# Jonetz/TreeDetection

Measured on AMD Instinct MI355X. Metric: tiles/sec (1000x1000 RGB+nDSM) predict_tiles model stage, higher is better.
Workload: dtype f32

## Files before the change

treedetection_amd/csrc/api.cpp:

```cpp
#include "common.h"
#include "detect.h"
#include <cstdarg>
#include <cstdio>
#include <cmath>
#include <cstdlib>
#include <vector>


namespace {
td_status scratch(void** p, size_t bytes) {
    TD_HIP_CHECK(hipMalloc(p, bytes ? bytes : 16));
    return TD_OK;
}
}

extern "C" {

void td_model_desc_default(td_model_desc* d) {
    d->num_classes = 1;
    d->precision = TD_PRECISION_FP32;
    d->pre_nms_topk = 1000;
    d->post_nms_topk = 1000;
    d->detections_per_image = 100;
    d->rpn_nms_thresh = 0.7f;
// ... 36 lines not shown
    a.stride = 1; a.pad = pad;
    a.Ho = H + 2 * pad - KH + 1;
    a.Wo = W + 2 * pad - KW + 1;
    a.relu = 1; a.M = B * a.Ho * a.Wo; a.m_mul = 1;
    a.tile_cfg = ((precision >> 8) & 0xff) - 1;
    TD_REQUIRE(conv_head_capable(a.tile_cfg, TD_PRECISION_FP16), "td_conv2d_head_nhwc: tile id %d does not own 256 output channels per block", a.tile_cfg);
    a.head_w = head_w; a.head_b = head_b; a.head_y = head_y; a.head_n = head_n;
    a.y = head_y;
    return conv2d_api(a, precision, stream);
}

static td_status conv2d_api(ConvArgs& a, int precision, void* stream) {
    hipStream_t s = static_cast<hipStream_t>(stream);
    ConvArgs with_frag = a;
    with_frag.w_frag = a.w;
    if (!conv_tile(a.tile_cfg) || !conv_tile(a.tile_cfg)->frag || conv_tile_refusal(a.tile_cfg, with_frag, precision & 0xff))
        return conv2d_launch(a, precision & 0xff, s);
    const int es = (precision & 0xff) == TD_PRECISION_FP16 ? 2 : 4;
    const size_t n = (size_t)a.Cout * a.KH * a.KW * a.Cin;
    std::vector<unsigned char> bits(n * es), packed;
    TD_HIP_CHECK(hipStreamSynchronize(s));
    TD_HIP_CHECK(hipMemcpy(bits.data(), a.w, n * es, hipMemcpyDeviceToHost));
    conv_bd_pack(bits.data(), es, a.Cout, a.KH, a.KW, a.Cin, packed);
    void* wf = nullptr;
    td_status st = scratch(&wf, packed.size());
    if (st < 0) return st;
    hipError_t herr = hipMemcpy(wf, packed.data(), packed.size(), hipMemcpyHostToDevice);
    a.w_frag = wf;
    if (herr == hipSuccess) st = conv2d_launch(a, precision & 0xff, s);
    hipError_t herr2 = hipStreamSynchronize(s);
// ... 212 lines not shown
```

treedetection_amd/csrc/common.h:

```cpp
#pragma once
#include <hip/hip_runtime.h>
#include <hip/hip_fp16.h>
#include <cstdint>
#include <cstddef>
#include "../../include/treedet.h"
#include <string>
#include <vector>

void td_set_error(const char* fmt, ...);

int td_polygons_json_text(const int32_t* mask_region, const int64_t* mask_offset, const uint32_t* mask_bits, int64_t mask_words,
                          const float* scores, const int32_t* classes, int n, const double* transform, const char* image_id,
                          std::string& out, const char* who);

#define TD_HIP_CHECK(expr)                                                                         \
    do {                                                                                           \
        hipError_t _e = (expr);                                                                    \
        if (_e != hipSuccess) {                                                                    \
            td_set_error("%s failed: %s (%s:%d)", #expr, hipGetErrorString(_e), __FILE__, __LINE__); \
            return TD_ERR_HIP;                                                                     \
        }                                                                                          \
    } while (0)

#define TD_REQUIRE(cond, ...)            \
// ... 17 lines not shown
    const float* bias;
    const void* res;
    void* y;
    int B, H, W, Cin, Cout, KH, KW, stride, pad, Ho, Wo;
    int res_shift;
    int relu;
    int out_mode;
    int M;
    const int* m_dyn;
    int m_mul;
    int m_off;
    int out_f32;
    int batch_count;
    long long x_bs, w_bs, y_bs;
    const void* w_frag;
    int tile_cfg;
    int tile_strict;
    const void* head_w;
    const float* head_b;
    float* head_y;
    int head_n;
    int nlev;
    struct Level {
        const void* x;
        const void* w;
        const float* bias;
        void* y;
        float* head_y;
        int H, W, M, tile0;
    } lev[5];
    int ntiles;
};
enum ConvFamily : unsigned char { TILE_IGEMM, TILE_PP8, TILE_PLANE, TILE_BD, TILE_BS, TILE_RETIRED };
enum : unsigned char { TILE_F32 = 1 << TD_PRECISION_FP32, TILE_F16 = 1 << TD_PRECISION_FP16, TILE_ANY = TILE_F32 | TILE_F16 };
struct ConvTile {
    ConvFamily family;
    unsigned char variant;
    unsigned char prec;
    bool head;
    bool frag;
    signed char tune_rank;
    unsigned char max_ksteps;
    short min_cout, max_cout;
};
inline constexpr ConvTile TD_CONV_TILES[] = {
    {TILE_IGEMM,   0, TILE_ANY, false, false,  5, 0,   0,  0},
    {TILE_IGEMM,   0, TILE_ANY, false, false, 10, 0,   0,  0},
    {TILE_IGEMM,   0, TILE_ANY, false, false, 11, 0,   0,  0},
// ... 16 lines not shown
    {TILE_PLANE,   0, TILE_F32, false, false, 19, 0,   0,  0},
    {TILE_PLANE,   0, TILE_F32, false, false, 20, 0,   0,  0},
    {TILE_RETIRED, 0, 0,        false, false, -1, 0,   0,  0},
    {TILE_RETIRED, 0, 0,        false, false, -1, 0,   0,  0},
    {TILE_BD,      0, TILE_ANY, true,  true,   8, 0,   0,  0},
    {TILE_BD,      1, TILE_ANY, false, true,  12, 0,   0,  0},
    {TILE_BD,      2, TILE_ANY, false, true,  13, 0,   0,  0},
    {TILE_BD,      3, TILE_ANY, false, true,  14, 0,   0,  0},
    {TILE_BD,      4, TILE_ANY, true,  true,   9, 0,   0,  0},
    {TILE_RETIRED, 0, 0,        false, false, -1, 0,   0,  0},
    {TILE_BD,      5, TILE_ANY, true,  true,   3, 0,   0,  0},
    {TILE_BD,      6, TILE_ANY, false, true,   7, 0,   0,  0},
    {TILE_IGEMM,   0, TILE_ANY, false, false, 15, 0,   0, 32},
    {TILE_IGEMM,   0, TILE_ANY, false, false, 17, 0,   0, 32},
    {TILE_BS,      0, TILE_ANY, false, true,   0, 4, 128,  0},
};
static inline const ConvTile* conv_tile(int id) { return id >= 0 && id < (int)(sizeof TD_CONV_TILES / sizeof *TD_CONV_TILES) ? &TD_CONV_TILES[id] : nullptr; }
static inline bool conv_head_capable(int id, int precision) { return precision == TD_PRECISION_FP16 && conv_tile(id) && conv_tile(id)->head; }
const char* conv_tile_refusal(int id, const ConvArgs& a, int precision);
td_status conv2d_launch(const ConvArgs& a, int precision, hipStream_t stream);
td_status conv_pp8_grouped_launch(ConvArgs a, hipStream_t stream);
void conv_bd_pack(const void* w_ohwi, int elem_bytes, int cout, int kh, int kw, int cin, std::vector<unsigned char>& out);
bool conv_bd_ok(const ConvArgs& a, int precision);
td_status conv_bd_launch(const ConvArgs& a, int precision, int variant, hipStream_t stream);
bool conv_bs_ok(const ConvArgs& a, int precision);
td_status conv_bs_launch(const ConvArgs& a, int precision, hipStream_t stream);
td_status wino_gemm_launch(const ConvArgs& a, hipStream_t stream);

struct TailArgs {
    const void* x;
    const void* w2;
    const float* scale2;
    const float* bias2;
    const void* w3;
    const float* scale3;
    const float* bias3;
    const void* res;
    void* y;
    int B, H, W, MID, COUT, M;
};
bool bottleneck_tail_ok(int precision, int mid, int cout);
// ... 38 lines not shown
```

treedetection_amd/csrc/conv_igemm.hip:

```cpp
#include "common.h"
#include <cstdlib>
#include <type_traits>

#include "conv_tiles.h"

namespace {

template <typename T, typename TO, int MT, int NT, int NSTAGE, int WM, int WN>
__global__ __launch_bounds__(64 * WM * WN, NSTAGE == 1 && MT * NT <= 4 ? 4 : 1)
void conv_igemm_kernel(const ConvArgs a_in) {
    ConvArgs a = a_in;
    if (a.batch_count > 1) {
        const long long bz = blockIdx.y;
        a.x = static_cast<const T*>(a.x) + bz * a.x_bs;
        a.w = static_cast<const T*>(a.w) + bz * a.w_bs;
        a.y = static_cast<TO*>(a.y) + bz * a.y_bs;
    }
    constexpr int THREADS = 64 * WM * WN;
    constexpr int BM = 32 * MT * WM, BN = 32 * NT * WN;
    constexpr int LDROWS = THREADS / 8;
    constexpr int AROWS = BM / LDROWS, BROWS = BN / LDROWS;
    static_assert(BM % LDROWS == 0 && BN % LDROWS == 0 && LDROWS % 16 == 0, "tile / thread-count mismatch");
    constexpr int ES = sizeof(T);
    constexpr int KE = Elem<T>::PER_CHUNK;
// ... 912 lines not shown
const char* conv_tile_refusal(int id, const ConvArgs& a, int precision) {
    const ConvTile* t = conv_tile(id);
    if (!t) return id < 0 ? nullptr : "no such tile id";
    if (t->family == TILE_RETIRED)
        return "a retired experiment (stream-K / the 4-wave 256x256 tile) that lost to the block tiles and left the library";
    const unsigned prec_bit = precision == TD_PRECISION_FP16 ? TILE_F16 : precision == TD_PRECISION_FP32 ? TILE_F32 : 0;
    if (!(t->prec & prec_bit)) return t->prec == TILE_F16 ? "fp16-only tile" : "fp32-only tile";
    if (t->family == TILE_PP8 && (a.out_mode != 0 || a.batch_count > 1)) return "plain output, no batched launch only";
    if (t->family == TILE_PLANE && !(a.KH == 1 && a.KW == 1 && a.stride == 1 && a.pad == 0 && a.out_mode == 0 && a.res_shift == 0 && !a.out_f32 &&
                                     a.m_off == 0 && a.Cin >= 32 && a.Cin % 32 == 0 && a.M > 0 && a.Cout > 0 && (a.batch_count <= 1 || !a.res) &&
                                     (size_t)a.M * a.Cin * 4 < 0xfffffff0ull - (1u << 20)))
        return "plane-only tile (fp32 1x1, stride 1, no padding, no upsampled residual, Cin a multiple of 32)";
    if (t->family == TILE_BS && !conv_bs_ok(a, precision))
        return "conv_bs_ok failed (1x1, stride 1, 1 / 2 / 4 k-chunks, 128 <= Cout <= 2048, Cout % 8 == 0, packed filters)";
    if (t->family == TILE_BD && !conv_bd_ok(a, precision)) return "conv_bd_ok failed (packed filters, plain output)";
    return nullptr;
}

td_status conv2d_launch(const ConvArgs& a, int precision, hipStream_t stream) {
    TD_REQUIRE(precision == TD_PRECISION_FP32 || precision == TD_PRECISION_FP16, "conv2d: bad precision %d", precision);
    int cfg = a.tile_cfg;
    if (cfg < 0) {
        const char* forced = getenv("TD_CONV_CFG");
        if (forced) cfg = atoi(forced);
    }
    if (const char* why = conv_tile_refusal(cfg, a, precision)) {
        if (a.tile_strict || !conv_tile(cfg) || conv_tile(cfg)->family == TILE_RETIRED) {
            td_set_error("conv2d: tile_cfg %d cannot run this launch%s: %s", cfg, a.tile_strict ? " (strict tile selection)" : "", why);
            return TD_ERR_INVALID;
        }
// ... 4 lines not shown
    TD_REQUIRE(a.M > 0 && a.Cout > 0, "conv2d: empty problem (M=%d, Cout=%d)", a.M, a.Cout);
    const size_t es = precision == TD_PRECISION_FP16 ? 2 : 4;
    TD_REQUIRE((size_t)a.B * a.H * a.W * (size_t)a.Cin * es < 0xfffffff0ull - (1u << 20), "conv2d: input tensor must stay below 4 GB (32-bit buffer offsets)");
    TD_REQUIRE((size_t)a.Cout * a.KH * a.KW * a.Cin * es < 0xfffffff0ull - (1u << 20), "conv2d: weight tensor must stay below 4 GB");
    TD_REQUIRE(a.KH * a.KW <= 32, "conv2d: at most 32 filter taps (got %dx%d)", a.KH, a.KW);
    TD_REQUIRE(a.out_mode == 0 || (a.Cout % 32 == 0 && !a.res), "conv2d: bad deconv configuration");
    TD_REQUIRE(!a.head_w || (conv_head_capable(cfg, precision) && a.Cout == 256 && !a.res && a.out_mode == 0 && a.head_y && a.head_n >= 1 && a.head_n <= 32),
               "conv2d: a fused head needs a 256-channel fp16 layer on a tile that owns all its channels (tile id %d)", cfg);
    if (cfg < 0) {
        const bool small_m = a.M <= 64 * 256;
        cfg = a.Cout <= 64 ? (small_m ? 3 : 1) : (small_m ? 2 : 0);
    }
    const ConvTile& t = *conv_tile(cfg);
    if (t.family == TILE_BS) return conv_bs_launch(a, precision, stream);
    if (t.family == TILE_BD) return conv_bd_launch(a, precision, t.variant, stream);
    TD_REQUIRE(a.batch_count <= 1 || (a.KH == 1 && a.KW == 1 && !a.res), "conv2d: batched launches are 1x1 contractions");
    if (t.family == TILE_PP8) return a.out_f32 ? pp8_launch<float>(a, stream) : pp8_launch<_Float16>(a, stream);
    if (t.family == TILE_PLANE) return plane_launch(a, cfg, stream);
    if (precision == TD_PRECISION_FP32) return dispatch<float, float>(a, cfg, stream);
    if (a.out_f32) return dispatch<_Float16, float>(a, cfg, stream);
    return dispatch<_Float16, _Float16>(a, cfg, stream);
}
```

treedetection_amd/csrc/engine.cpp:

```cpp
#include "common.h"
#include "detect.h"

#include <cmath>
#include <cstdio>
#include <cstdlib>
#include <cstring>
#include <algorithm>
#include <functional>
#include <map>
#include <optional>
#include <string>
#include <tuple>
#include <vector>

namespace {

struct HostTensor {
    const float* data = nullptr;
    std::vector<int64_t> shape;
    int64_t numel() const {
        int64_t n = 1;
        for (auto s : shape) n *= s;
        return n;
    }
};

struct ConvLayer {
    int cout = 0, cin = 0, kh = 1, kw = 1;
    void* w = nullptr;
    float* scale = nullptr;
    float* bias = nullptr;
    bool out_f32 = false;
    void* w_frag = nullptr;
    float* wino_u = nullptr;
    float* wino_u43 = nullptr;
};

struct Block {
    ConvLayer c1, c2, c3, sc;
    bool has_sc = false;
    int stride = 1;
};

struct NamedTensor {
    void* p = nullptr;
    int64_t dims[4] = {0, 0, 0, 0};
    int elem = 4;
};
// ... 53 lines not shown
    bool autotune = true;
    int backbone_subbatch = 0;
    std::map<std::tuple<int, int, int, int, int>, int> tuned;
    bool winograd = true;
    float *wino_v = nullptr, *wino_m = nullptr;
    size_t wino_elems = 0;
    bool group_levels = true;
    bool fuse_head = true;
    bool fuse_tail = true;
    bool fuse_tail_fp16 = false;
    bool wino_fused = true;
    int wino_slab = 0;
    int wino_minc = 128;
    int wino43_min = 12;
    int wino_fold = 39;
    std::string tune_cache;
    void* tune_evict = nullptr;
    size_t tune_evict_bytes = 0;

    struct FwdCtx {
        const void* images = nullptr;
        int input_format = 0, B = 0, Hp = 0, Wp = 0;
        ImgSizes valid{}, outsz{};
        td_detections out{};
        bool valid_ctx = false;
    } ctx;
    hipEvent_t phase_ev[7] = {};
    bool phase_ev_recorded[7] = {};
    hipEvent_t prev5_ev = nullptr;
    bool prev5_recorded = false;
// ... 60 lines not shown
    if (off || L.cin % ke != 0 || L.kh * L.kw > 32 || (size_t)L.cout * L.kh * L.kw * L.cin != h.size()) return TD_OK;
    std::vector<unsigned char> packed;
    if (f16) {
        std::vector<unsigned short> bits(h.size());
        for (size_t i = 0; i < h.size(); ++i) bits[i] = __builtin_bit_cast(unsigned short, (_Float16)h[i]);
        conv_bd_pack(bits.data(), 2, L.cout, L.kh, L.kw, L.cin, packed);
    } else {
        conv_bd_pack(h.data(), 4, L.cout, L.kh, L.kw, L.cin, packed);
    }
    unsigned char* d = nullptr;
    td_status st = upload(e, packed, &d);
    L.w_frag = d;
    return st;
}

using TensorMap = std::map<std::string, HostTensor>;

td_status need(const TensorMap& tm, const std::string& name, int ndim, const HostTensor** out) {
    auto it = tm.find(name);
    if (it == tm.end()) {
        td_set_error("load_weights: tensor '%s' missing", name.c_str());
        return TD_ERR_WEIGHTS;
    }
    if ((int)it->second.shape.size() != ndim) {
        td_set_error("load_weights: tensor '%s' has %d dims, expected %d", name.c_str(), (int)it->second.shape.size(), ndim);
        return TD_ERR_WEIGHTS;
    }
    *out = &it->second;
    return TD_OK;
}
// ... 38 lines not shown
}

td_status upload_wino(td_engine* e, const std::vector<float>& w_ohwi, ConvLayer& L) {
    L.wino_u = nullptr;
    if (e->desc.precision != TD_PRECISION_FP32 || !e->winograd || L.kh != 3 || L.kw != 3 || L.cin % 32 != 0 || L.cout % 4 != 0)
        return TD_OK;
    std::vector<float> u((size_t)16 * L.cout * L.cin);
    wino_filter_transform(w_ohwi.data(), L.cout, L.cin, u.data());
    td_status st = upload(e, u, &L.wino_u);
    if (st < 0 || e->wino43_min <= 0 || L.cin < e->wino_minc || L.cout < e->wino_minc) return st;
    std::vector<float> u43((size_t)36 * L.cout * L.cin);
    wino43_filter_transform(w_ohwi.data(), L.cout, L.cin, u43.data());
    return upload(e, u43, &L.wino_u43);
}

td_status load_conv_bn(td_engine* e, const TensorMap& tm, const std::string& p, ConvLayer& L) {
    const HostTensor* w;
    td_status st = need(tm, p + ".weight", 4, &w);
    if (st < 0) return st;
    L.cout = (int)w->shape[0];
    L.cin = (int)w->shape[1];
    L.kh = (int)w->shape[2];
    L.kw = (int)w->shape[3];
    const std::vector<float> packed = pack_ohwi(*w);
    if ((st = upload_w(e, packed, &L.w)) < 0) return st;
    if ((st = upload_frag(e, packed, L)) < 0) return st;
    if ((st = upload_wino(e, packed, L)) < 0) return st;
    std::vector<float> s, b;
    if ((st = bn_fold(tm, p, L.cout, s, b)) < 0) return st;
    if ((st = upload(e, s, &L.scale)) < 0) return st;
    return upload(e, b, &L.bias);
}

td_status load_conv_bias(td_engine* e, const TensorMap& tm, const std::string& p, ConvLayer& L) {
    const HostTensor *w, *b;
    td_status st = need(tm, p + ".weight", 4, &w);
    if (st < 0) return st;
    if ((st = need(tm, p + ".bias", 1, &b)) < 0) return st;
    L.cout = (int)w->shape[0];
    L.cin = (int)w->shape[1];
    L.kh = (int)w->shape[2];
    L.kw = (int)w->shape[3];
    if (b->shape[0] != L.cout) {
        td_set_error("load_weights: bias of '%s' has wrong length", p.c_str());
        return TD_ERR_WEIGHTS;
    }
    const std::vector<float> packed = pack_ohwi(*w);
    if ((st = upload_w(e, packed, &L.w)) < 0) return st;
    if ((st = upload_frag(e, packed, L)) < 0) return st;
    if ((st = upload_wino(e, packed, L)) < 0) return st;
    L.scale = nullptr;
    return upload(e, std::vector<float>(b->data, b->data + L.cout), &L.bias);
}

void set_named(td_engine* e, const char* name, void* p, int64_t d0, int64_t d1 = 0, int64_t d2 = 0, int64_t d3 = 0,
               int elem = 4) {
    NamedTensor t;
    t.p = p;
    t.dims[0] = d0; t.dims[1] = d1; t.dims[2] = d2; t.dims[3] = d3;
    t.elem = elem;
    e->named[name] = t;
}

hipEvent_t prof_event(td_engine* e) {
// ... 92 lines not shown
    TD_HIP_CHECK(hipGetDeviceCount(&ndev));
    TD_REQUIRE(device >= 0 && device < ndev, "td_engine_create: device %d of %d", device, ndev);
    TD_HIP_CHECK(hipSetDevice(device));
    td_engine* e = new td_engine();
    if (const char* sbenv = getenv("TD_BACKBONE_SUBBATCH")) e->backbone_subbatch = atoi(sbenv);
    if (const char* tc = getenv("TD_TUNE_CACHE")) e->tune_cache = tc;
    if (const char* wg = getenv("TD_WINOGRAD")) e->winograd = atoi(wg) != 0;
    if (const char* ws = getenv("TD_WINO_SLAB")) e->wino_slab = atoi(ws);
    if (const char* wf = getenv("TD_WINO_FUSED")) e->wino_fused = atoi(wf) != 0;
    if (const char* fh = getenv("TD_FUSE_HEAD")) e->fuse_head = atoi(fh) != 0;
    if (const char* gl = getenv("TD_GROUP_LEVELS")) e->group_levels = atoi(gl) != 0;
    if (const char* ft = getenv("TD_FUSE_TAIL")) { e->fuse_tail = atoi(ft) != 0; e->fuse_tail_fp16 = atoi(ft) == 2; }
    if (const char* w4 = getenv("TD_WINO43_MIN")) e->wino43_min = atoi(w4);
    if (const char* wf2 = getenv("TD_WINO_FOLD")) e->wino_fold = atoi(wf2);
    if (const char* wc = getenv("TD_WINO_MINC")) e->wino_minc = atoi(wc);
    e->desc = d;
    load_tune_cache(e);
    e->device = device;
    *out = e;
    return TD_OK;
}

void td_engine_destroy(td_engine* e) {
    if (!e) return;
    (void)hipSetDevice(e->device);
    free_pool(e->weight_allocs);
    free_pool(e->ws_allocs);
    if (e->tune_evict) (void)hipFree(e->tune_evict);
    for (auto& r : e->prof_recs) { (void)hipEventDestroy(r.a); (void)hipEventDestroy(r.b); }
    for (auto& r : e->cls_recs) { (void)hipEventDestroy(r.a); (void)hipEventDestroy(r.b); }
// ... 41 lines not shown
        if (e->desc.precision == TD_PRECISION_FP16 && e->stem_c == 64 && !(mfma_stem && atoi(mfma_stem) == 0)) {
            std::vector<unsigned short> w16;
            std::vector<float> b16;
            stem_mfma_prepare(p.data(), s.data(), b.data(), e->stem_c, w16, b16);
            if ((st = upload(e, w16, &e->stem_w16)) < 0) return st;
            if ((st = upload(e, b16, &e->stem_bias16)) < 0) return st;
        }
    }
    for (int si = 0; si < 4; ++si) {
        e->stages[si].clear();
        for (int bi = 0;; ++bi) {
            const std::string p = "backbone.bottom_up.res" + std::to_string(si + 2) + "." + std::to_string(bi);
            if (tm.find(p + ".conv1.weight") == tm.end()) break;
            Block blk;
            blk.stride = (bi == 0 && si > 0) ? 2 : 1;
            if ((st = load_conv_bn(e, tm, p + ".conv1", blk.c1)) < 0) return st;
            if ((st = load_conv_bn(e, tm, p + ".conv2", blk.c2)) < 0) return st;
            if ((st = load_conv_bn(e, tm, p + ".conv3", blk.c3)) < 0) return st;
            blk.has_sc = tm.find(p + ".shortcut.weight") != tm.end();
            if (blk.has_sc && (st = load_conv_bn(e, tm, p + ".shortcut", blk.sc)) < 0) return st;
            e->stages[si].push_back(blk);
        }
        if (e->stages[si].empty()) {
            td_set_error("load_weights: no blocks found for res%d", si + 2);
            return TD_ERR_WEIGHTS;
        }
    }
    for (int l = 0; l < 4; ++l) {
        if ((st = load_conv_bias(e, tm, "backbone.fpn_lateral" + std::to_string(l + 2), e->lateral[l])) < 0) return st;
        if ((st = load_conv_bias(e, tm, "backbone.fpn_output" + std::to_string(l + 2), e->fpn_out[l])) < 0) return st;
    }
    e->fpn_c = e->lateral[0].cout;
    if ((st = load_conv_bias(e, tm, "proposal_generator.rpn_head.conv", e->rpn_conv)) < 0) return st;
    {
        const HostTensor *wo, *bo, *wd, *bd;
        if ((st = need(tm, "proposal_generator.rpn_head.objectness_logits.weight", 4, &wo)) < 0) return st;
        if ((st = need(tm, "proposal_generator.rpn_head.objectness_logits.bias", 1, &bo)) < 0) return st;
        if ((st = need(tm, "proposal_generator.rpn_head.anchor_deltas.weight", 4, &wd)) < 0) return st;
        if ((st = need(tm, "proposal_generator.rpn_head.anchor_deltas.bias", 1, &bd)) < 0) return st;
        if (wo->shape[0] != RPN_A || wd->shape[0] != 4 * RPN_A || wo->shape[1] != e->fpn_c || wd->shape[1] != e->fpn_c) {
            td_set_error("load_weights: RPN head must have %d anchors per position", RPN_A);
            return TD_ERR_WEIGHTS;
        }
        const int c = e->fpn_c;
// ... 13 lines not shown
        if ((st = need(tm, "roi_heads.box_head.fc1.weight", 2, &w)) < 0) return st;
        if ((st = need(tm, "roi_heads.box_head.fc1.bias", 1, &b)) < 0) return st;
        const int c = e->fpn_c, o = (int)w->shape[0];
        if (w->shape[1] != (int64_t)c * 49) {
            td_set_error("load_weights: fc1 expects %d inputs", c * 49);
            return TD_ERR_WEIGHTS;
        }
        std::vector<float> p((size_t)o * c * 49);
        for (int r = 0; r < o; ++r)
            for (int ch = 0; ch < c; ++ch)
                for (int q = 0; q < 49; ++q) p[(size_t)r * c * 49 + (size_t)q * c + ch] = w->data[(size_t)r * c * 49 + (size_t)ch * 49 + q];
        e->fc1.cout = o; e->fc1.cin = c * 49; e->fc1.kh = e->fc1.kw = 1;
        e->fc_dim = o;
        if ((st = upload_w(e, p, &e->fc1.w)) < 0) return st;
        if ((st = upload_frag(e, p, e->fc1)) < 0) return st;
        if ((st = upload(e, std::vector<float>(b->data, b->data + o), &e->fc1.bias)) < 0) return st;
    }
    {
        const HostTensor *w, *b;
        if ((st = need(tm, "roi_heads.box_head.fc2.weight", 2, &w)) < 0) return st;
        if ((st = need(tm, "roi_heads.box_head.fc2.bias", 1, &b)) < 0) return st;
        e->fc2.cout = (int)w->shape[0]; e->fc2.cin = (int)w->shape[1]; e->fc2.kh = e->fc2.kw = 1;
        const std::vector<float> w2v(w->data, w->data + w->numel());
        if ((st = upload_w(e, w2v, &e->fc2.w)) < 0) return st;
        if ((st = upload_frag(e, w2v, e->fc2)) < 0) return st;
        if ((st = upload(e, std::vector<float>(b->data, b->data + e->fc2.cout), &e->fc2.bias)) < 0) return st;
    }
    {
        const HostTensor *wc, *bc, *wr, *br;
        if ((st = need(tm, "roi_heads.box_predictor.cls_score.weight", 2, &wc)) < 0) return st;
        if ((st = need(tm, "roi_heads.box_predictor.cls_score.bias", 1, &bc)) < 0) return st;
        if ((st = need(tm, "roi_heads.box_predictor.bbox_pred.weight", 2, &wr)) < 0) return st;
        if ((st = need(tm, "roi_heads.box_predictor.bbox_pred.bias", 1, &br)) < 0) return st;
        if (wc->shape[0] != 2 || wr->shape[0] != 4) {
            td_set_error("load_weights: box predictor must be 1 class (+background), got cls %lld / reg %lld rows",
                         (long long)wc->shape[0], (long long)wr->shape[0]);
            return TD_ERR_WEIGHTS;
        }
        const int k = (int)wc->shape[1];
        std::vector<float> w((size_t)6 * k), b(6);
// ... 177 lines not shown
        float t = 0.f;
        TD_HIP_CHECK(hipEventElapsedTime(&t, ea, eb));
        t /= (float)reps;
        if (t < ms) ms = t;
        if (!cold && ms > 0.1f) break;
    }
    *ms_out = ms;
    return TD_OK;
}

td_status tuned_cfg(td_engine* e, const std::tuple<int, int, int, int, int>& key, int prec, const ConvArgs& a, hipStream_t s,
                    const std::function<td_status(int)>& launch_cfg, int* cfg_out) {
    const int ksteps = a.KH * a.KW * a.Cin / (prec == TD_PRECISION_FP16 ? 64 : 32);
    auto candidate = [&](int id) {
        const ConvTile* t = conv_tile(id);
        return t && (!t->max_ksteps || ksteps <= t->max_ksteps) && a.Cout >= t->min_cout && (!t->max_cout || a.Cout <= t->max_cout) &&
               !conv_tile_refusal(id, a, prec);
    };
    static const int forced = getenv("TD_FORCE_CFG") ? atoi(getenv("TD_FORCE_CFG")) : -1;
    if (candidate(forced)) {
        *cfg_out = forced;
        return TD_OK;
    }
    auto it = e->tuned.find(key);
    if (it == e->tuned.end()) {
        load_tune_cache(e);
        it = e->tuned.find(key);
    }
    if (it != e->tuned.end()) {
        *cfg_out = it->second;
        return TD_OK;
// ... 132 lines not shown
            ClassScope cs(e, s_, TD_CLS_WINO_XFORM, hflops, mb + hb);
            return wino43_output_head_launch(e->wino_m, B_, H_, W_, L.cout, L.scale, L.bias, relu ? 1 : 0, static_cast<const float*>(head->w),
                                             head->bias, head_y, head->cout, s_);
        }
        ClassScope cs(e, s_, dyn ? TD_CLS_MASK_HEAD : TD_CLS_WINO_XFORM, 0.0, dyn ? 0.0 : mb + yb);
        return wino43_output_launch(e->wino_m, B_, H_, W_, L.cout, L.scale, L.bias, relu ? 1 : 0, static_cast<float*>(y_), m_dyn, s_);
    };
    auto run_conv = [&](const ConvLayer& L, const void* x_, int B_, int H_, int W_, int stride, int pad, bool relu,
                        void* y_, const void* res_, int res_shift, hipStream_t s_, int prec_,
                        const int* m_dyn = nullptr, int m_mul = 1, int out_mode = 0,
                        const ConvLayer* head = nullptr, float* head_y = nullptr, bool* head_fused = nullptr) -> td_status {
        const int Ho = (H_ + 2 * pad - L.kh) / stride + 1, Wo = (W_ + 2 * pad - L.kw) / stride + 1;
        const double M = (double)B_ * Ho * Wo, K = (double)L.kh * L.kw * L.cin;
        const double flops = 2.0 * M * L.cout * K;
        const double es = prec_ == TD_PRECISION_FP16 ? 2.0 : 4.0;
        const double bytes = es * ((double)B_ * H_ * W_ * L.cin / (stride * stride) + M * L.cout * (res_ ? 2.0 : 1.0) + L.cout * K);
        int cfg = -1, wino_cfg = -1;
        bool use_wino = false, use_43 = false, use_fold = false;
        td_status st2;
        ConvArgs ca{};
        ca.x = x_; ca.w = L.w; ca.w_frag = L.w_frag; ca.scale = L.scale; ca.bias = L.bias; ca.res = res_; ca.y = y_;
        ca.B = B_; ca.H = H_; ca.W = W_; ca.Cin = L.cin; ca.Cout = L.cout; ca.KH = L.kh; ca.KW = L.kw;
        ca.stride = stride; ca.pad = pad; ca.Ho = Ho; ca.Wo = Wo;
        ca.res_shift = res_shift; ca.relu = relu ? 1 : 0; ca.out_mode = out_mode;
        ca.M = B_ * Ho * Wo; ca.m_dyn = m_dyn; ca.m_mul = m_mul; ca.tile_cfg = -1; ca.out_f32 = L.out_f32 ? 1 : 0;
        if (e->autotune) {
            const auto key = std::make_tuple(L.cout, L.cin, L.kh * 16 + L.kw, B_ * Ho * Wo, stride * 4 + out_mode * 2 + (res_ ? 1 : 0));
            auto direct = [&](int c) { ConvArgs a = ca; a.tile_cfg = c; return conv2d_launch(a, prec_, s_); };
            const bool wino_ok = prec_ == TD_PRECISION_FP32 && L.wino_u && e->wino_v && stride == 1 && pad == 1 && !res_ && out_mode == 0 &&
                                 (!m_dyn || ((H_ | W_) & 1) == 0) &&
                                 (size_t)16 * std::min<long long>((long long)B_ * ((H_ + 1) / 2) * ((W_ + 1) / 2), wino_slab_tiles(e, L)) *
                                         (size_t)std::max(L.cin, L.cout) <= e->wino_elems;
            if (wino_ok) {
                const int T = (int)std::min<long long>((long long)B_ * ((H_ + 1) / 2) * ((W_ + 1) / 2), wino_slab_tiles(e, L));
                const auto wkey = std::make_tuple(L.cout, L.cin, 1 * 16 + 1, T, 4 + 32);
                auto wino = [&](int c) { return run_wino(L, x_, B_, H_, W_, relu, y_, s_, m_dyn, m_mul, c); };
                use_wino = L.cin >= e->wino_minc && L.cout >= e->wino_minc;
                const long long T43 = (long long)B_ * ((H_ + 3) / 4) * ((W_ + 3) / 4);
                use_43 = use_wino && L.wino_u43 && e->wino43_min > 0 && H_ >= e->wino43_min && W_ >= e->wino43_min &&
                         (size_t)36 * T43 * (size_t)std::max(L.cin, L.cout) <= e->wino_elems && T43 * std::max(L.cin, L.cout) < (1ll << 31);
                const int hw_ = H_ * W_, wf_ = e->wino_fold;
                use_fold = use_43 && wf_ > 0 && wino43_fused_ok(m_dyn ? B_ : 1, H_, W_, L.cin, L.cout) &&
// ... 1 lines not shown
                            ((wf_ & 2) && m_dyn && !head) || ((wf_ & 4) && !m_dyn && !head && L.cin == 256 && hw_ >= 80 * 80) ||
                            ((wf_ & 8) && !m_dyn && !head && hw_ >= 40 * 40) || ((wf_ & 16) && !m_dyn && !head));
                if (use_43 && !use_fold) {
                    const auto key43 = std::make_tuple(L.cout, L.cin, 1 * 16 + 1, (int)T43, 4 + 64);
                    auto w43 = [&](int c) { return run_wino43(L, x_, B_, H_, W_, relu, y_, s_, m_dyn, c); };
                    if ((st2 = tuned_cfg(e, key43, prec_, wino43_plane_args(e, L, B_, H_, W_, m_dyn), s_, w43, &wino_cfg)) < 0) return st2;
                }
                if (use_wino && !use_43 && !e->wino_fused &&
                    (st2 = tuned_cfg(e, wkey, prec_, wino_plane_args(e, L, x_, B_, H_, W_, T, 0, m_dyn, m_mul), s_, wino, &wino_cfg)) < 0) return st2;
            }
            if (!use_wino && (st2 = tuned_cfg(e, key, prec_, ca, s_, direct, &cfg)) < 0) return st2;
        }
        ProfScope ps(e, s_, m_dyn ? 7 : 0, m_dyn ? 0.0 : flops, m_dyn ? 0.0 : bytes);
        if (e->prof && !m_dyn) {
            const double padded = use_43 ? (double)(((H_ + 3) / 4) * 4) * (((W_ + 3) / 4) * 4) / ((double)H_ * W_) : 1.0;
            e->prof_flops[8] += use_43 ? flops * padded * 0.25 : (use_wino ? flops * 4.0 / 9.0 : flops);
            e->prof_launches[8] += use_wino ? 1 : 0;
        }
        if (use_43) {
            const bool fuse43 = head && !use_fold && e->fuse_head && !m_dyn && relu && L.cout == 256 && head->cin == 256 && head->kh == 1 && head->kw == 1 &&
                                head->cout <= 32 && !head->scale;
            if (head_fused) *head_fused = fuse43;
            return run_wino43(L, x_, B_, H_, W_, relu, y_, s_, m_dyn, wino_cfg, fuse43 ? head : nullptr, fuse43 ? head_y : nullptr, use_fold);
        }
        if (use_wino) return run_wino(L, x_, B_, H_, W_, relu, y_, s_, m_dyn, m_mul, wino_cfg);
        const int cls = m_dyn ? TD_CLS_MASK_HEAD : (H_ == 1 && W_ == 1 ? TD_CLS_FC : (L.kh == 1 && L.kw == 1 ? TD_CLS_CONV1X1 : TD_CLS_CONV3X3));
        const bool fuse_head = head && e->fuse_head && !m_dyn && out_mode == 0 && !res_ && relu && L.cout == 256 && head->cin == 256 &&
                               head->kh == 1 && head->kw == 1 && head->cout <= 32 && head->out_f32 && !head->scale && conv_head_capable(cfg, prec_);
        if (head_fused) *head_fused = fuse_head;
        ca.tile_cfg = cfg;
        if (fuse_head) {
            const double hflops = 2.0 * M * head->cout * L.cout, hbytes = 4.0 * M * head->cout + es * head->cout * L.cout;
            const double bytes_f = bytes - es * M * L.cout + hbytes;
            if (e->prof) {
                e->prof_flops[0] += hflops;
                e->prof_flops[8] += hflops;
                e->prof_launches[0] += 1;
                e->prof_bytes[0] += hbytes + es * M * L.cout;
            }
            ca.head_w = head->w; ca.head_b = head->bias; ca.head_y = head_y; ca.head_n = head->cout;
            ClassScope cs(e, s_, cls, flops + hflops, bytes_f);
            return conv2d_launch(ca, prec_, s_);
        }
        ClassScope cs(e, s_, cls, m_dyn ? 0.0 : flops, m_dyn ? 0.0 : bytes);
        return conv2d_launch(ca, prec_, s_);
    };
    auto groupable = [&](const ConvLayer& L) {
        return L.kh == 3 && L.kw == 3 && L.cout == 256 && L.cin % 64 == 0 && !L.scale && L.bias && !L.out_f32;
    };
    auto run_grouped = [&](const ConvLayer* const* Ls, const void* const* xs, void* const* ys, float* const* head_ys, int nl, const int* Hs,
                           const int* Ws, bool relu, const ConvLayer* head, hipStream_t s_) -> td_status {
        ConvArgs a{};
        a.B = B; a.Cin = Ls[0]->cin; a.Cout = 256; a.KH = a.KW = 3; a.stride = 1; a.pad = 1; a.relu = relu ? 1 : 0; a.m_mul = 1; a.nlev = nl;
        a.tile_cfg = 17;
        double flops = 0.0, bytes = 0.0, unfused_bytes = 0.0;
        for (int l = 0; l < nl; ++l) {
            a.lev[l].x = xs[l]; a.lev[l].w = Ls[l]->w; a.lev[l].bias = Ls[l]->bias;
            a.lev[l].y = ys ? ys[l] : nullptr; a.lev[l].head_y = head_ys ? head_ys[l] : nullptr;
            a.lev[l].H = Hs[l]; a.lev[l].W = Ws[l];
// ... 462 lines not shown
```

Baseline: 664.6.

## Add split-bf16 MFMA kernel for fp32 1x1 convolutions and FC layers

Adds a new conv family that emulates fp32 1x1 contractions by splitting each operand into three bf16 terms and accumulating six bf16 MFMA products. The filters are pre-split and packed at load time, and activations are split on the fly from LDS. The engine routes FC layers to it by default, with an env mask to also cover lateral, conv1, conv3 and shortcut layers. The aim is to use the bf16 matrix cores instead of slower fp32 paths for these contractions. The trade-off is extra VALU work for splitting, six MMAs per product, and a small accuracy difference from true fp32.

```diff
diff --git a/treedetection_amd/csrc/api.cpp b/treedetection_amd/csrc/api.cpp
--- a/treedetection_amd/csrc/api.cpp
+++ b/treedetection_amd/csrc/api.cpp
@@ -74,6 +74,27 @@
     hipStream_t s = static_cast<hipStream_t>(stream);
     ConvArgs with_frag = a;
     with_frag.w_frag = a.w;
+    with_frag.w_split = a.w;
+    if (conv_tile(a.tile_cfg) && conv_tile(a.tile_cfg)->family == TILE_SPLIT && !conv_tile_refusal(a.tile_cfg, with_frag, precision & 0xff)) {
+        const size_t n = (size_t)a.Cout * a.Cin;
+        std::vector<float> wh(n);
+        std::vector<unsigned char> packed;
+        TD_HIP_CHECK(hipStreamSynchronize(s));
+        TD_HIP_CHECK(hipMemcpy(wh.data(), a.w, n * sizeof(float), hipMemcpyDeviceToHost));
+        conv_split_pack(wh.data(), a.Cout, a.Cin, packed);
+        void* ws = nullptr;
+        td_status st = scratch(&ws, packed.size());
+        if (st < 0) return st;
+        hipError_t herr = hipMemcpy(ws, packed.data(), packed.size(), hipMemcpyHostToDevice);
+        a.w_split = ws;
+        if (herr == hipSuccess) st = conv2d_launch(a, precision & 0xff, s);
+        hipError_t herr2 = hipStreamSynchronize(s);
+        (void)hipFree(ws);
+        if (st < 0) return st;
+        TD_HIP_CHECK(herr);
+        TD_HIP_CHECK(herr2);
+        return TD_OK;
+    }
     if (!conv_tile(a.tile_cfg) || !conv_tile(a.tile_cfg)->frag || conv_tile_refusal(a.tile_cfg, with_frag, precision & 0xff))
         return conv2d_launch(a, precision & 0xff, s);
     const int es = (precision & 0xff) == TD_PRECISION_FP16 ? 2 : 4;
diff --git a/treedetection_amd/csrc/common.h b/treedetection_amd/csrc/common.h
--- a/treedetection_amd/csrc/common.h
+++ b/treedetection_amd/csrc/common.h
@@ -55,6 +55,7 @@
     int batch_count;
     long long x_bs, w_bs, y_bs;
     const void* w_frag;
+    const void* w_split;
     int tile_cfg;
     int tile_strict;
     const void* head_w;
@@ -72,7 +73,7 @@
     } lev[5];
     int ntiles;
 };
-enum ConvFamily : unsigned char { TILE_IGEMM, TILE_PP8, TILE_PLANE, TILE_BD, TILE_BS, TILE_RETIRED };
+enum ConvFamily : unsigned char { TILE_IGEMM, TILE_PP8, TILE_PLANE, TILE_BD, TILE_BS, TILE_RETIRED, TILE_SPLIT };
 enum : unsigned char { TILE_F32 = 1 << TD_PRECISION_FP32, TILE_F16 = 1 << TD_PRECISION_FP16, TILE_ANY = TILE_F32 | TILE_F16 };
 struct ConvTile {
     ConvFamily family;
@@ -119,6 +120,9 @@
     {TILE_IGEMM,   0, TILE_ANY, false, false, 15, 0,   0, 32},
     {TILE_IGEMM,   0, TILE_ANY, false, false, 17, 0,   0, 32},
     {TILE_BS,      0, TILE_ANY, false, true,   0, 4, 128,  0},
+    {TILE_SPLIT,   0, TILE_F32, false, false, 21, 0,   0,  0},
+    {TILE_SPLIT,   1, TILE_F32, false, false, 22, 0,   0,  0},
+    {TILE_SPLIT,   2, TILE_F32, false, false, 23, 0,   0,  0},
 };
 static inline const ConvTile* conv_tile(int id) { return id >= 0 && id < (int)(sizeof TD_CONV_TILES / sizeof *TD_CONV_TILES) ? &TD_CONV_TILES[id] : nullptr; }
 static inline bool conv_head_capable(int id, int precision) { return precision == TD_PRECISION_FP16 && conv_tile(id) && conv_tile(id)->head; }
@@ -130,6 +134,9 @@
 td_status conv_bd_launch(const ConvArgs& a, int precision, int variant, hipStream_t stream);
 bool conv_bs_ok(const ConvArgs& a, int precision);
 td_status conv_bs_launch(const ConvArgs& a, int precision, hipStream_t stream);
+void conv_split_pack(const float* w, int cout, int cin, std::vector<unsigned char>& out);
+bool conv_split_ok(const ConvArgs& a, int precision);
+td_status conv_split_launch(const ConvArgs& a, int variant, hipStream_t stream);
 td_status wino_gemm_launch(const ConvArgs& a, hipStream_t stream);
 
 struct TailArgs {
diff --git a/treedetection_amd/csrc/conv_igemm.hip b/treedetection_amd/csrc/conv_igemm.hip
--- a/treedetection_amd/csrc/conv_igemm.hip
+++ b/treedetection_amd/csrc/conv_igemm.hip
@@ -950,6 +950,8 @@
     if (t->family == TILE_BS && !conv_bs_ok(a, precision))
         return "conv_bs_ok failed (1x1, stride 1, 1 / 2 / 4 k-chunks, 128 <= Cout <= 2048, Cout % 8 == 0, packed filters)";
     if (t->family == TILE_BD && !conv_bd_ok(a, precision)) return "conv_bd_ok failed (packed filters, plain output)";
+    if (t->family == TILE_SPLIT && !conv_split_ok(a, precision))
+        return "conv_split_ok failed (fp32 1x1 without padding, plain output, Cin a multiple of 32, split filter bank)";
     return nullptr;
 }
 
@@ -984,6 +986,7 @@
     const ConvTile& t = *conv_tile(cfg);
     if (t.family == TILE_BS) return conv_bs_launch(a, precision, stream);
     if (t.family == TILE_BD) return conv_bd_launch(a, precision, t.variant, stream);
+    if (t.family == TILE_SPLIT) return conv_split_launch(a, t.variant, stream);
     TD_REQUIRE(a.batch_count <= 1 || (a.KH == 1 && a.KW == 1 && !a.res), "conv2d: batched launches are 1x1 contractions");
     if (t.family == TILE_PP8) return a.out_f32 ? pp8_launch<float>(a, stream) : pp8_launch<_Float16>(a, stream);
     if (t.family == TILE_PLANE) return plane_launch(a, cfg, stream);
diff --git a/treedetection_amd/csrc/conv_split.hip b/treedetection_amd/csrc/conv_split.hip
--- /dev/null
+++ b/treedetection_amd/csrc/conv_split.hip
@@ -0,0 +1,250 @@
+#include "common.h"
+#include "conv_tiles.h"
+
+namespace {
+
+typedef __bf16 bf16x8 __attribute__((ext_vector_type(8)));
+typedef __bf16 bf16x2 __attribute__((ext_vector_type(2)));
+typedef float f32x2 __attribute__((ext_vector_type(2)));
+typedef unsigned u32x4 __attribute__((ext_vector_type(4)));
+
+constexpr int SPLIT_CHUNK_BYTES = 6144;
+
+__device__ __forceinline__ void split8(const f32x4& lo, const f32x4& hi, bf16x8 (&p)[3]) {
+    u32x4 w[3];
+#pragma unroll
+    for (int e = 0; e < 4; ++e) {
+        f32x2 v = e < 2 ? f32x2{lo[2 * e], lo[2 * e + 1]} : f32x2{hi[2 * e - 4], hi[2 * e - 3]};
+#pragma unroll
+        for (int k = 0; k < 3; ++k) {
+            const unsigned u = __builtin_bit_cast(unsigned, __builtin_convertvector(v, bf16x2));
+            w[k][e] = u;
+            if (k < 2) {
+                const f32x2 back = {__builtin_bit_cast(float, u << 16), __builtin_bit_cast(float, u & 0xffff0000u)};
+                v = v - back;
+            }
+        }
+    }
+#pragma unroll
+    for (int k = 0; k < 3; ++k) p[k] = __builtin_bit_cast(bf16x8, w[k]);
+}
+
+template <int MT, int NT, int WM, int WN>
+__device__ __forceinline__ void conv_split_body(const ConvArgs& a, char* lds) {
+    constexpr int THREADS = 64 * WM * WN;
+    constexpr int BM = 32 * MT * WM, BN = 32 * NT * WN;
+    constexpr int LDROWS = THREADS / 8;
+    constexpr int AROWS = BM / LDROWS;
+    static_assert(BM % LDROWS == 0 && AROWS >= 1 && LDROWS % 16 == 0, "tile / thread-count mismatch");
+    char* As = lds;
+
+    int M = a.M;
+    if (a.m_dyn) {
+        int md = *a.m_dyn * a.m_mul - a.m_off;
+        md = md < 0 ? 0 : md;
+        M = md < M ? md : M;
+    }
+    const int tiles_n = (a.Cout + BN - 1) / BN;
+    const int tiles_m = (M + BM - 1) / BM;
+    const int nblk = tiles_m * tiles_n;
+    if ((int)blockIdx.x >= nblk) return;
+    const int pid = xcd_remap(blockIdx.x, nblk);
+    const int tm = pid / tiles_n, tn = pid - tm * tiles_n;
+    const int m0 = tm * BM, n0 = tn * BN;
+
+    const int tid = threadIdx.x;
+    const int lane = tid & 63, wave = tid >> 6;
+    const int wm = wave / WN, wn = wave - wm * WN;
+    const int ld_c = tid & 7, ld_r = tid >> 3;
+    const int nit = a.Cin / 32;
+    const unsigned pix_bytes = (unsigned)a.Cin * 4u;
+    const __amdgpu_buffer_rsrc_t xrsrc = __builtin_amdgcn_make_buffer_rsrc(
+        const_cast<void*>(a.x), 0, (int)((size_t)a.B * a.H * a.W * pix_bytes), 0x00020000);
+    const int ntiles32 = (a.Cout + 31) / 32;
+    const __amdgpu_buffer_rsrc_t wrsrc = __builtin_amdgcn_make_buffer_rsrc(
+        const_cast<void*>(a.w_split), 0, (int)((size_t)ntiles32 * nit * SPLIT_CHUNK_BYTES), 0x00020000);
+    constexpr unsigned OOB = 0xfffffff0u;
+    const unsigned src_piece = (unsigned)(ld_c ^ ((ld_r >> 1) & 7)) * 16;
+
+    unsigned a_off[AROWS];
+#pragma unroll
+    for (int i = 0; i < AROWS; ++i) {
+        const int m = m0 + ld_r + LDROWS * i;
+        a_off[i] = OOB;
+        if (m < M && a.stride == 1) {
+            a_off[i] = (unsigned)m * pix_bytes + src_piece;
+        } else if (m < M) {
+            const int hw = a.Ho * a.Wo;
+            const int b = m / hw;
+            const int rem = m - b * hw;
+            const int oy = rem / a.Wo;
+            const int ox = rem - oy * a.Wo;
+            a_off[i] = (unsigned)((b * a.H + oy * a.stride) * a.W + ox * a.stride) * pix_bytes + src_piece;
+        }
+    }
+    unsigned w_off[NT];
+#pragma unroll
+    for (int j = 0; j < NT; ++j) {
+        const int nt = n0 / 32 + wn * NT + j;
+        w_off[j] = nt < ntiles32 ? (unsigned)nt * (unsigned)nit * (unsigned)SPLIT_CHUNK_BYTES + (unsigned)lane * 16u : OOB;
+    }
+
+    typedef __attribute__((address_space(3))) void lds_void;
+    const unsigned wave_rows = (unsigned)__builtin_amdgcn_readfirstlane(wave) * 8u;
+    auto stage_a = [&](int stage, int it) {
+#pragma unroll
+        for (int i = 0; i < AROWS; ++i) {
+            const unsigned off = a_off[i] == OOB || it >= nit ? OOB : a_off[i] + (unsigned)it * CHUNK_BYTES;
+            char* dst = As + ((unsigned)stage * BM + (unsigned)LDROWS * i + wave_rows) * CHUNK_BYTES;
+            __builtin_amdgcn_raw_ptr_buffer_load_lds(xrsrc, (lds_void*)dst, 16, off, 0, 0, 0);
+        }
+    };
+    auto load_b = [&](f32x4 (&fb)[NT][3], int it, int sl) {
+#pragma unroll
+        for (int j = 0; j < NT; ++j)
+#pragma unroll
+            for (int q = 0; q < 3; ++q) {
+                const unsigned off = w_off[j] == OOB || it >= nit ? OOB : w_off[j] + (unsigned)it * (unsigned)SPLIT_CHUNK_BYTES + (unsigned)(3 * sl + q) * 1024u;
+                fb[j][q] = __builtin_bit_cast(f32x4, __builtin_amdgcn_raw_buffer_load_b128(wrsrc, off, 0, 0));
+            }
+    };
+
+    f32x16 acc[MT][NT];
+#pragma unroll
+    for (int i = 0; i < MT; ++i)
+#pragma unroll
+        for (int j = 0; j < NT; ++j)
+#pragma unroll
+            for (int r = 0; r < 16; ++r) acc[i][j][r] = 0.f;
+    const unsigned swz = (lane >> 1) & 7, hi = lane >> 5;
+    unsigned frag_off[4];
+#pragma unroll
+    for (int kk = 0; kk < 4; ++kk)
+        frag_off[kk] = (unsigned)(wm * 32 * MT + (lane & 31)) * CHUNK_BYTES + (((unsigned)(2 * kk) + hi) ^ swz) * 16;
+    auto split_a = [&](int stage, int sl, bf16x8 (&pa)[MT][3]) {
+        const char* Ab = &As[stage * BM * CHUNK_BYTES];
+#pragma unroll
+        for (int i = 0; i < MT; ++i) {
+            const f32x4 lo = *reinterpret_cast<const f32x4*>(Ab + i * 32 * CHUNK_BYTES + frag_off[2 * sl]);
+            const f32x4 up = *reinterpret_cast<const f32x4*>(Ab + i * 32 * CHUNK_BYTES + frag_off[2 * sl + 1]);
+            split8(lo, up, pa[i]);
+        }
+    };
+    auto mma = [&](const bf16x8 (&pa)[MT][3], const f32x4 (&fb)[NT][3]) {
+        constexpr int PA[6] = {0, 2, 1, 0, 1, 0}, QB[6] = {2, 0, 1, 1, 0, 0};
+#pragma unroll
+        for (int t = 0; t < 6; ++t)
+#pragma unroll
+            for (int i = 0; i < MT; ++i)
+#pragma unroll
+                for (int j = 0; j < NT; ++j)
+                    acc[i][j] = __builtin_amdgcn_mfma_f32_32x32x16_bf16(pa[i][PA[t]], __builtin_bit_cast(bf16x8, fb[j][QB[t]]), acc[i][j], 0, 0, 0);
+    };
+
+    constexpr int A_YOUNGER = 3 * NT * 3 + AROWS;
+    static_assert(A_YOUNGER < 64, "vmcnt immediate");
+    f32x4 fb[3][NT][3];
+    bf16x8 pa[2][MT][3];
+    stage_a(0, 0);
+    stage_a(1, 1);
+    stage_a(2, 2);
+    load_b(fb[0], 0, 0);
+    load_b(fb[1], 0, 1);
+    asm volatile("s_waitcnt vmcnt(0)" ::: "memory");
+    __builtin_amdgcn_s_barrier();
+    split_a(0, 0, pa[0]);
+    auto step = [&](auto c_c, auto s_c, int it) {
+        constexpr int C = decltype(c_c)::value, S = decltype(s_c)::value, G = 2 * C + S;
+        if constexpr (S == 1) {
+            asm volatile("s_waitcnt vmcnt(%0)" ::"n"(A_YOUNGER) : "memory");
+            asm volatile("s_waitcnt lgkmcnt(0)" ::: "memory");
+            __builtin_amdgcn_s_barrier();
+        }
+        load_b(fb[(G + 2) % 3], it + 1, S);
+        if constexpr (S == 1) stage_a(C, it + 3);
+        __builtin_amdgcn_sched_barrier(0);
+        if constexpr (S == 0) split_a(C, 1, pa[1]);
+        else split_a((C + 1) % 3, 0, pa[0]);
+        mma(pa[S], fb[G % 3]);
+    };
+    for (int it = 0; it < nit; it += 3) {
+        step(std::integral_constant<int, 0>{}, std::integral_constant<int, 0>{}, it);
+        step(std::integral_constant<int, 0>{}, std::integral_constant<int, 1>{}, it);
+        if (it + 1 < nit) {
+            step(std::integral_constant<int, 1>{}, std::integral_constant<int, 0>{}, it + 1);
+            step(std::integral_constant<int, 1>{}, std::integral_constant<int, 1>{}, it + 1);
+        }
+        if (it + 2 < nit) {
+            step(std::integral_constant<int, 2>{}, std::integral_constant<int, 0>{}, it + 2);
+            step(std::integral_constant<int, 2>{}, std::integral_constant<int, 1>{}, it + 2);
+        }
+    }
+    asm volatile("s_waitcnt vmcnt(0)" ::: "memory");
+    asm volatile("s_waitcnt lgkmcnt(0)" ::: "memory");
+    __builtin_amdgcn_s_barrier();
+    conv_epilogue<float, float, MT, NT, WM, WN, 1>(a, acc, lds, M, m0, n0, tid, lane, wm, wn);
+}
+
+template <int MT, int NT, int WM, int WN, int WPE>
+__global__ __launch_bounds__(64 * WM * WN, WPE)
+void conv_split_kernel(const ConvArgs a) {
+    constexpr int STAGE_BYTES = 3 * 32 * MT * WM * CHUNK_BYTES;
+    constexpr int EPI_BYTES = conv_epilogue_lds_bytes<float, MT, NT, WM, WN, 1>();
+    constexpr int LDS_BYTES = STAGE_BYTES > EPI_BYTES ? STAGE_BYTES : EPI_BYTES;
+    static_assert(LDS_BYTES <= 80 * 1024, "two blocks per CU must fit the LDS");
+    __shared__ __attribute__((aligned(16))) char lds[LDS_BYTES];
+    conv_split_body<MT, NT, WM, WN>(a, lds);
+}
+
+template <int MT, int NT, int WM, int WN, int WPE>
+td_status launch_split(const ConvArgs& a, hipStream_t stream) {
+    const int tiles = td_cdiv(a.M, 32 * MT * WM) * td_cdiv(a.Cout, 32 * NT * WN);
+    hipLaunchKernelGGL((conv_split_kernel<MT, NT, WM, WN, WPE>), dim3(tiles), dim3(64 * WM * WN), 0, stream, a);
+    TD_KERNEL_CHECK();
+    return TD_OK;
+}
+
+inline unsigned short bf16_rne(float f) {
+    unsigned u = __builtin_bit_cast(unsigned, f);
+    if ((u & 0x7fffffffu) > 0x7f800000u) return (unsigned short)((u >> 16) | 0x40);
+    u += 0x7fffu + ((u >> 16) & 1u);
+    return (unsigned short)(u >> 16);
+}
+
+}
+
+void conv_split_pack(const float* w, int cout, int cin, std::vector<unsigned char>& out) {
+    const int nit = cin / 32, nt32 = (cout + 31) / 32;
+    out.assign((size_t)nt32 * nit * SPLIT_CHUNK_BYTES, (unsigned char)0);
+    unsigned short* o = reinterpret_cast<unsigned short*>(out.data());
+    for (int t = 0; t < nt32; ++t)
+        for (int c = 0; c < nit; ++c)
+            for (int s = 0; s < 2; ++s)
+                for (int l = 0; l < 64; ++l) {
+                    const int n = t * 32 + (l & 31), h = l >> 5;
+                    if (n >= cout) continue;
+                    for (int e = 0; e < 8; ++e) {
+                        float v = w[(size_t)n * cin + (size_t)c * 32 + 16 * s + 8 * (e >> 2) + 4 * h + (e & 3)];
+                        for (int p = 0; p < 3; ++p) {
+                            const unsigned short b = bf16_rne(v);
+                            o[(((((size_t)t * nit + c) * 2 + s) * 3 + p) * 64 + l) * 8 + e] = b;
+                            v = v - __builtin_bit_cast(float, (unsigned)b << 16);
+                        }
+                    }
+                }
+}
+
+bool conv_split_ok(const ConvArgs& a, int precision) {
+    return precision == TD_PRECISION_FP32 && a.w_split && a.KH == 1 && a.KW == 1 && a.pad == 0 && a.stride >= 1 && a.out_mode == 0 &&
+           a.batch_count <= 1 && !a.out_f32 && !a.head_w && a.Cin >= 32 && a.Cin % 32 == 0 &&
+           (size_t)((a.Cout + 31) / 32) * (size_t)(a.Cin / 32) * SPLIT_CHUNK_BYTES < 0xfffffff0ull - (1u << 20);
+}
+
+td_status conv_split_launch(const ConvArgs& a, int variant, hipStream_t stream) {
+    TD_REQUIRE(conv_split_ok(a, TD_PRECISION_FP32), "split-bf16 contraction: unsupported launch (fp32 1x1 without padding, split filter bank)");
+    switch (variant) {
+        case 2: return launch_split<2, 4, 1, 2, 1>(a, stream);
+        case 1: return launch_split<2, 2, 2, 2, 2>(a, stream);
+        default: return launch_split<2, 4, 2, 2, 1>(a, stream);
+    }
+}
diff --git a/treedetection_amd/csrc/engine.cpp b/treedetection_amd/csrc/engine.cpp
--- a/treedetection_amd/csrc/engine.cpp
+++ b/treedetection_amd/csrc/engine.cpp
@@ -25,6 +25,8 @@
     }
 };
 
+enum { SPLIT_FC = 1, SPLIT_LATERAL = 2, SPLIT_CONV1 = 4, SPLIT_CONV3 = 8, SPLIT_SHORTCUT = 16, SPLIT_DEFAULT = SPLIT_FC };
+
 struct ConvLayer {
     int cout = 0, cin = 0, kh = 1, kw = 1;
     void* w = nullptr;
@@ -32,6 +34,7 @@
     float* bias = nullptr;
     bool out_f32 = false;
     void* w_frag = nullptr;
+    void* w_split = nullptr;
     float* wino_u = nullptr;
     float* wino_u43 = nullptr;
 };
@@ -115,6 +118,7 @@
     int wino_minc = 128;
     int wino43_min = 12;
     int wino_fold = 39;
+    int f32_split = SPLIT_DEFAULT;
     std::string tune_cache;
     void* tune_evict = nullptr;
     size_t tune_evict_bytes = 0;
@@ -205,6 +209,19 @@
     return st;
 }
 
+td_status upload_split(td_engine* e, const std::vector<float>& h, ConvLayer& L, int cls) {
+    L.w_split = nullptr;
+    if (e->desc.precision != TD_PRECISION_FP32 || !(e->f32_split & cls) || L.kh != 1 || L.kw != 1 || L.cin < 256 || L.cin % 32 != 0 ||
+        (size_t)L.cout * L.cin != h.size())
+        return TD_OK;
+    std::vector<unsigned char> packed;
+    conv_split_pack(h.data(), L.cout, L.cin, packed);
+    unsigned char* d = nullptr;
+    td_status st = upload(e, packed, &d);
+    L.w_split = d;
+    return st;
+}
+
 using TensorMap = std::map<std::string, HostTensor>;
 
 td_status need(const TensorMap& tm, const std::string& name, int ndim, const HostTensor** out) {
@@ -273,7 +290,7 @@
     return upload(e, u43, &L.wino_u43);
 }
 
-td_status load_conv_bn(td_engine* e, const TensorMap& tm, const std::string& p, ConvLayer& L) {
+td_status load_conv_bn(td_engine* e, const TensorMap& tm, const std::string& p, ConvLayer& L, int split_cls = 0) {
     const HostTensor* w;
     td_status st = need(tm, p + ".weight", 4, &w);
     if (st < 0) return st;
@@ -284,6 +301,7 @@
     const std::vector<float> packed = pack_ohwi(*w);
     if ((st = upload_w(e, packed, &L.w)) < 0) return st;
     if ((st = upload_frag(e, packed, L)) < 0) return st;
+    if ((st = upload_split(e, packed, L, split_cls)) < 0) return st;
     if ((st = upload_wino(e, packed, L)) < 0) return st;
     std::vector<float> s, b;
     if ((st = bn_fold(tm, p, L.cout, s, b)) < 0) return st;
@@ -291,7 +309,7 @@
     return upload(e, b, &L.bias);
 }
 
-td_status load_conv_bias(td_engine* e, const TensorMap& tm, const std::string& p, ConvLayer& L) {
+td_status load_conv_bias(td_engine* e, const TensorMap& tm, const std::string& p, ConvLayer& L, int split_cls = 0) {
     const HostTensor *w, *b;
     td_status st = need(tm, p + ".weight", 4, &w);
     if (st < 0) return st;
@@ -307,6 +325,7 @@
     const std::vector<float> packed = pack_ohwi(*w);
     if ((st = upload_w(e, packed, &L.w)) < 0) return st;
     if ((st = upload_frag(e, packed, L)) < 0) return st;
+    if ((st = upload_split(e, packed, L, split_cls)) < 0) return st;
     if ((st = upload_wino(e, packed, L)) < 0) return st;
     L.scale = nullptr;
     return upload(e, std::vector<float>(b->data, b->data + L.cout), &L.bias);
@@ -429,6 +448,7 @@
     if (const char* w4 = getenv("TD_WINO43_MIN")) e->wino43_min = atoi(w4);
     if (const char* wf2 = getenv("TD_WINO_FOLD")) e->wino_fold = atoi(wf2);
     if (const char* wc = getenv("TD_WINO_MINC")) e->wino_minc = atoi(wc);
+    if (const char* sp = getenv("TD_F32_SPLIT")) e->f32_split = atoi(sp);
     e->desc = d;
     load_tune_cache(e);
     e->device = device;
@@ -500,11 +520,11 @@
             if (tm.find(p + ".conv1.weight") == tm.end()) break;
             Block blk;
             blk.stride = (bi == 0 && si > 0) ? 2 : 1;
-            if ((st = load_conv_bn(e, tm, p + ".conv1", blk.c1)) < 0) return st;
+            if ((st = load_conv_bn(e, tm, p + ".conv1", blk.c1, si > 0 ? SPLIT_CONV1 : 0)) < 0) return st;
             if ((st = load_conv_bn(e, tm, p + ".conv2", blk.c2)) < 0) return st;
-            if ((st = load_conv_bn(e, tm, p + ".conv3", blk.c3)) < 0) return st;
+            if ((st = load_conv_bn(e, tm, p + ".conv3", blk.c3, si > 0 ? SPLIT_CONV3 : 0)) < 0) return st;
             blk.has_sc = tm.find(p + ".shortcut.weight") != tm.end();
-            if (blk.has_sc && (st = load_conv_bn(e, tm, p + ".shortcut", blk.sc)) < 0) return st;
+            if (blk.has_sc && (st = load_conv_bn(e, tm, p + ".shortcut", blk.sc, si > 0 ? SPLIT_SHORTCUT : 0)) < 0) return st;
             e->stages[si].push_back(blk);
         }
         if (e->stages[si].empty()) {
@@ -513,7 +533,7 @@
         }
     }
     for (int l = 0; l < 4; ++l) {
-        if ((st = load_conv_bias(e, tm, "backbone.fpn_lateral" + std::to_string(l + 2), e->lateral[l])) < 0) return st;
+        if ((st = load_conv_bias(e, tm, "backbone.fpn_lateral" + std::to_string(l + 2), e->lateral[l], SPLIT_LATERAL)) < 0) return st;
         if ((st = load_conv_bias(e, tm, "backbone.fpn_output" + std::to_string(l + 2), e->fpn_out[l])) < 0) return st;
     }
     e->fpn_c = e->lateral[0].cout;
@@ -557,6 +577,7 @@
         e->fc_dim = o;
         if ((st = upload_w(e, p, &e->fc1.w)) < 0) return st;
         if ((st = upload_frag(e, p, e->fc1)) < 0) return st;
+        if ((st = upload_split(e, p, e->fc1, SPLIT_FC)) < 0) return st;
         if ((st = upload(e, std::vector<float>(b->data, b->data + o), &e->fc1.bias)) < 0) return st;
     }
     {
@@ -567,6 +588,7 @@
         const std::vector<float> w2v(w->data, w->data + w->numel());
         if ((st = upload_w(e, w2v, &e->fc2.w)) < 0) return st;
         if ((st = upload_frag(e, w2v, e->fc2)) < 0) return st;
+        if ((st = upload_split(e, w2v, e->fc2, SPLIT_FC)) < 0) return st;
         if ((st = upload(e, std::vector<float>(b->data, b->data + e->fc2.cout), &e->fc2.bias)) < 0) return st;
     }
     {
@@ -774,7 +796,7 @@
     const int ksteps = a.KH * a.KW * a.Cin / (prec == TD_PRECISION_FP16 ? 64 : 32);
     auto candidate = [&](int id) {
         const ConvTile* t = conv_tile(id);
-        return t && (!t->max_ksteps || ksteps <= t->max_ksteps) && a.Cout >= t->min_cout && (!t->max_cout || a.Cout <= t->max_cout) &&
+        return t && (t->family == TILE_SPLIT) == (a.w_split != nullptr) && (!t->max_ksteps || ksteps <= t->max_ksteps) && a.Cout >= t->min_cout && (!t->max_cout || a.Cout <= t->max_cout) &&
                !conv_tile_refusal(id, a, prec);
     };
     static const int forced = getenv("TD_FORCE_CFG") ? atoi(getenv("TD_FORCE_CFG")) : -1;
@@ -937,18 +959,19 @@
         const double M = (double)B_ * Ho * Wo, K = (double)L.kh * L.kw * L.cin;
         const double flops = 2.0 * M * L.cout * K;
         const double es = prec_ == TD_PRECISION_FP16 ? 2.0 : 4.0;
-        const double bytes = es * ((double)B_ * H_ * W_ * L.cin / (stride * stride) + M * L.cout * (res_ ? 2.0 : 1.0) + L.cout * K);
-        int cfg = -1, wino_cfg = -1;
+        const bool split = L.w_split && prec_ == TD_PRECISION_FP32 && out_mode == 0 && !m_dyn && !head && pad == 0;
+        const double bytes = es * ((double)B_ * H_ * W_ * L.cin / (stride * stride) + M * L.cout * (res_ ? 2.0 : 1.0)) + (split ? 6.0 : es) * L.cout * K;
+        int cfg = split ? 34 : -1, wino_cfg = -1;
         bool use_wino = false, use_43 = false, use_fold = false;
         td_status st2;
         ConvArgs ca{};
-        ca.x = x_; ca.w = L.w; ca.w_frag = L.w_frag; ca.scale = L.scale; ca.bias = L.bias; ca.res = res_; ca.y = y_;
+        ca.x = x_; ca.w = L.w; ca.w_frag = L.w_frag; ca.w_split = split ? L.w_split : nullptr; ca.scale = L.scale; ca.bias = L.bias; ca.res = res_; ca.y = y_;
         ca.B = B_; ca.H = H_; ca.W = W_; ca.Cin = L.cin; ca.Cout = L.cout; ca.KH = L.kh; ca.KW = L.kw;
         ca.stride = stride; ca.pad = pad; ca.Ho = Ho; ca.Wo = Wo;
         ca.res_shift = res_shift; ca.relu = relu ? 1 : 0; ca.out_mode = out_mode;
         ca.M = B_ * Ho * Wo; ca.m_dyn = m_dyn; ca.m_mul = m_mul; ca.tile_cfg = -1; ca.out_f32 = L.out_f32 ? 1 : 0;
         if (e->autotune) {
-            const auto key = std::make_tuple(L.cout, L.cin, L.kh * 16 + L.kw, B_ * Ho * Wo, stride * 4 + out_mode * 2 + (res_ ? 1 : 0));
+            const auto key = std::make_tuple(L.cout, L.cin, L.kh * 16 + L.kw, B_ * Ho * Wo, stride * 4 + out_mode * 2 + (res_ ? 1 : 0) + (split ? 128 : 0));
             auto direct = [&](int c) { ConvArgs a = ca; a.tile_cfg = c; return conv2d_launch(a, prec_, s_); };
             const bool wino_ok = prec_ == TD_PRECISION_FP32 && L.wino_u && e->wino_v && stride == 1 && pad == 1 && !res_ && out_mode == 0 &&
                                  (!m_dyn || ((H_ | W_) & 1) == 0) &&
@@ -980,7 +1003,7 @@
         ProfScope ps(e, s_, m_dyn ? 7 : 0, m_dyn ? 0.0 : flops, m_dyn ? 0.0 : bytes);
         if (e->prof && !m_dyn) {
             const double padded = use_43 ? (double)(((H_ + 3) / 4) * 4) * (((W_ + 3) / 4) * 4) / ((double)H_ * W_) : 1.0;
-            e->prof_flops[8] += use_43 ? flops * padded * 0.25 : (use_wino ? flops * 4.0 / 9.0 : flops);
+            e->prof_flops[8] += use_43 ? flops * padded * 0.25 : (use_wino ? flops * 4.0 / 9.0 : (split ? flops * 6.0 / 16.0 : flops));
             e->prof_launches[8] += use_wino ? 1 : 0;
         }
         if (use_43) {
@@ -1008,7 +1031,7 @@
             ClassScope cs(e, s_, cls, flops + hflops, bytes_f);
             return conv2d_launch(ca, prec_, s_);
         }
-        ClassScope cs(e, s_, cls, m_dyn ? 0.0 : flops, m_dyn ? 0.0 : bytes);
+        ClassScope cs(e, s_, cls, m_dyn ? 0.0 : (split ? flops * 6.0 / 16.0 : flops), m_dyn ? 0.0 : bytes);
         return conv2d_launch(ca, prec_, s_);
     };
     auto groupable = [&](const ConvLayer& L) {
```

Measured after the change: 688.2 (median of 6 runs). +3.6%, better.
